# chrischoy/DeepGlobalRegistration

Hardware: NVIDIA H100
Metric: scan_pairs_per_sec (higher is better)
Workload: dtype f32

## Files before the change

deepglobalregistration_b200/csrc/spconv_ring.h:

```cpp
#pragma once

#if defined(__CUDACC__)
#define DGR_RING_HD __host__ __device__ __forceinline__
#else
#define DGR_RING_HD inline
#endif

namespace spconv_ring {

constexpr int kStages = 2;
constexpr int kIdxSlots = kStages + 1;
constexpr int kMaxRun = 8;

DGR_RING_HD int stage_of(unsigned g) { return (int)(g % kStages); }
DGR_RING_HD unsigned full_parity(unsigned g) { return (g / kStages) & 1u; }
DGR_RING_HD unsigned empty_parity(unsigned g) { return (g / kStages - 1u) & 1u; }
DGR_RING_HD int idx_slot(unsigned tile) { return (int)(tile % kIdxSlots); }

constexpr int kMinWaves = 2;
DGR_RING_HD int tile_run(int n_tiles, int resident) {
  const int r = n_tiles / (kMinWaves * (resident > 0 ? resident : 1));
  return r < 1 ? 1 : (r > kMaxRun ? kMaxRun : r);
}

}
```

deepglobalregistration_b200/csrc/spconv_tc.cu:

```cuda
#include <stdlib.h>

#include "common.cuh"
#include "spconv_ring.h"
#include "tc_common.cuh"

namespace {

using namespace tc;
using namespace spconv_ring;

#define DGR_TRY_RC(expr)             \
  do {                              \
    int32_t rc__ = (expr);          \
    if (rc__ != DGR_OK) return rc__; \
  } while (0)

constexpr int kConsumerWarps = 8;
constexpr int kProducerThreads = 128;
constexpr int kThreadsTC = kConsumerWarps * 32 + kProducerThreads;
constexpr int kTileM = 128;
constexpr int kChunk = 32;
constexpr int kATileBytes = kTileM * 128;
constexpr int kGatherRows = kTileM / (kProducerThreads / 8);
static_assert(kMaxRun <= 32, "one warp lists the tiles of a run");

struct TileDesc {
  int kappa, p0, rows;
};

struct TcShared {
  unsigned long long full[kStages];
  unsigned long long empty[kStages];
  int n_run;
  TileDesc tiles[kMaxRun];
  int out_rows[kIdxSlots][kTileM];
};

constexpr bool tc_line_epilogue(int nt) { return nt >= 128; }
constexpr int kScratchLd = 40;
constexpr int kScratchBytes = 16 * kScratchLd * 4;

constexpr size_t tc_smem_bytes(int nt) {
  return sizeof(TcShared) + 1024 + (size_t)kStages * (2 * kATileBytes + 2 * nt * 128) +
         (tc_line_epilogue(nt) ? (size_t)kConsumerWarps * kScratchBytes : 0);
}

constexpr int tc_min_ctas(int nt, bool f16) { return nt >= 128 || f16 ? 1 : 2; }
constexpr int kProducerRegs = 104, kConsumerRegs = 200;

template <int NT, bool kF16, int kPasses>
__global__ void __launch_bounds__(kThreadsTC, tc_min_ctas(NT, kF16))
spconv_tc_kernel(const float* __restrict__ in_feat, int cin, const unsigned char* __restrict__ wt, int cout,
                 const int32_t* __restrict__ in_idx, const int32_t* __restrict__ out_idx,
                 const int32_t* __restrict__ kofs, const int32_t* __restrict__ tile_k,
                 const int32_t* __restrict__ tile_start, int n_tiles, int run, const float* __restrict__ amax_in,
                 const float* __restrict__ w_inv_scale, float* __restrict__ out) {
  constexpr int kCh = kF16 ? 64 : kChunk;
  constexpr int kV = kF16 ? 2 : 1;
  constexpr int kBatches = kV, kBatchRows = kGatherRows / kBatches;
  constexpr int kBTileBytes = NT * 128;
  constexpr int kStageBytes = 2 * kATileBytes + 2 * kBTileBytes;
  extern __shared__ __align__(16) unsigned char smem_dyn[];
  TcShared& sh = *reinterpret_cast<TcShared*>(smem_dyn);
  unsigned char* stage0 = reinterpret_cast<unsigned char*>(
      (reinterpret_cast<uintptr_t>(smem_dyn) + sizeof(TcShared) + 1023) & ~(uintptr_t)1023);
  const int t = threadIdx.x, warp = __shfl_sync(0xffffffffu, t >> 5, 0), lane = t & 31;
  const int n_chunks = cin / kCh;
  const uint32_t b_tile_bytes = (uint32_t)cout * 128;
  const uint32_t slab_bytes = 2 * b_tile_bytes;
  const uint32_t full0 = smem_u32(&sh.full[0]), empty0 = smem_u32(&sh.empty[0]);

  if (t == 0) {
    for (int s = 0; s < kStages; ++s) {
      mbar_init(full0 + 8 * s, kProducerThreads + 1);
      mbar_init(empty0 + 8 * s, kConsumerWarps);
    }
    asm volatile("fence.mbarrier_init.release.cluster;" ::: "memory");
  }
  if (NT > cout) {
    const int pad_pieces = (NT - cout) * 8;
    for (int i = t; i < kStages * 2 * pad_pieces; i += kThreadsTC) {
      const int tile = i / pad_pieces, e = i % pad_pieces;
      *reinterpret_cast<uint4*>(stage0 + (tile >> 1) * kStageBytes + 2 * kATileBytes + (tile & 1) * kBTileBytes +
                                (cout + (e >> 3)) * 128 + (e & 7) * 16) = make_uint4(0u, 0u, 0u, 0u);
    }
  }
  if (warp == 0) {
    const int tile = blockIdx.x * run + lane;
    TileDesc d = {0, 0, 0};
    if (lane < run && tile < n_tiles) {
      d.kappa = tile_k[tile];
      d.p0 = tile_start[tile];
      d.rows = min(kTileM, kofs[d.kappa + 1] - d.p0);
    }
    const unsigned live = __ballot_sync(0xffffffffu, d.rows > 0);
    if (d.rows > 0) sh.tiles[__popc(live & ((1u << lane) - 1u))] = d;
    if (lane == 0) sh.n_run = __popc(live);
  }
  __syncthreads();
  const int n_run = sh.n_run;
  if (n_run == 0) return;

  if (warp >= kConsumerWarps) {
    if (NT >= 128) asm volatile("setmaxnreg.dec.sync.aligned.u32 %0;" ::"n"(kProducerRegs));
    const int pt = t - kConsumerWarps * 32, piece = pt & 7, rgrp = pt >> 3;
    const uint32_t a_off = (uint32_t)(rgrp * 128 + ((piece ^ (rgrp & 7)) << 4));
    const float sx = kF16 ? f16_scale_for(__ldg(amax_in)) : 1.f;
    auto load_idx = [&](int ti, int (&src)[kGatherRows], int& oj) {
      const TileDesc d = sh.tiles[ti < n_run ? ti : 0];
      const int rows = ti < n_run ? d.rows : 0;
#pragma unroll
      for (int i = 0; i < kGatherRows; ++i) {
        const int r = i * 16 + rgrp;
        src[i] = r < rows ? __ldg(in_idx + d.p0 + r) : -1;
      }
      oj = pt < rows ? __ldg(out_idx + d.p0 + pt) : -1;
    };
    int src[kGatherRows], src_next[kGatherRows], oj, oj_next;
    float4 v[kBatchRows][kV];
    auto load_a = [&](int c, int h) {
#pragma unroll
      for (int i = 0; i < kBatchRows; ++i)
#pragma unroll
        for (int u = 0; u < kV; ++u) {
          const int row = src[h * kBatchRows + i];
          v[i][u] = row >= 0 ? __ldg(reinterpret_cast<const float4*>(in_feat + (size_t)row * cin + c * kCh +
                                                                      piece * (4 * kV) + 4 * u))
                             : make_float4(0.f, 0.f, 0.f, 0.f);
        }
    };
    load_idx(0, src, oj);
    load_idx(1, src_next, oj_next);
    load_a(0, 0);
    unsigned g = 0;
    for (int ti = 0; ti < n_run; ++ti) {
      const unsigned char* slab = wt + (size_t)sh.tiles[ti].kappa * n_chunks * slab_bytes;
      for (int c = 0; c < n_chunks; ++c, ++g) {
        const int s = stage_of(g);
        unsigned char* a_hi = stage0 + (size_t)s * kStageBytes;
        unsigned char* a_lo = a_hi + kATileBytes;
        unsigned char* b_hi = a_lo + kATileBytes;
        if (g >= kStages) mbar_wait(empty0 + 8 * s, empty_parity(g));
        if (pt == 0) {
          const unsigned char* bsrc = slab + (size_t)c * slab_bytes;
          mbar_arrive_expect_tx(full0 + 8 * s, kPasses == 3 ? slab_bytes : b_tile_bytes);
          bulk_g2s(smem_u32(b_hi), bsrc, b_tile_bytes, full0 + 8 * s);
          if (kPasses == 3) bulk_g2s(smem_u32(b_hi + kBTileBytes), bsrc + b_tile_bytes, b_tile_bytes, full0 + 8 * s);
        }
        if (c == 0) sh.out_rows[idx_slot(ti)][pt] = oj;
#pragma unroll
        for (int h = 0; h < kBatches; ++h) {
#pragma unroll
          for (int i = 0; i < kBatchRows; ++i) {
            const uint32_t off = a_off + (h * kBatchRows + i) * 2048;
            if (kF16) split_store_f16(v[i][0], v[i][kV - 1], sx, a_hi, a_lo, off);
            else split_store(v[i][0], a_hi, a_lo, off);
          }
          if (h + 1 < kBatches) {
            load_a(c, h + 1);
          } else if (c + 1 < n_chunks) {
            load_a(c + 1, 0);
          } else if (ti + 1 < n_run) {
#pragma unroll
            for (int i = 0; i < kGatherRows; ++i) src[i] = src_next[i];
            oj = oj_next;
            load_a(0, 0);
            load_idx(ti + 2, src_next, oj_next);
          }
        }
        fence_proxy_async();
        mbar_arrive(full0 + 8 * s);
      }
    }
    return;
  }

  if (NT >= 128) asm volatile("setmaxnreg.inc.sync.aligned.u32 %0;" ::"n"(kConsumerRegs));
  const int wg = warp >> 2;
  const int r0 = wg * 64 + (warp & 3) * 16 + (lane >> 2);
  const float inv = kF16 ? __ldg(w_inv_scale) / f16_scale_for(__ldg(amax_in)) : 1.f;
  auto release = [&](unsigned gq) {
    __syncwarp();
    if (lane == 0) mbar_arrive(empty0 + 8 * stage_of(gq));
  };
  unsigned g = 0;
  for (int ti = 0; ti < n_run; ++ti) {
    float acc[NT / 2];
#pragma unroll
    for (int i = 0; i < NT / 2; ++i) acc[i] = 0.f;
    for (int c = 0; c < n_chunks; ++c, ++g) {
      const uint32_t a_hi = smem_u32(stage0 + (size_t)stage_of(g) * kStageBytes);
      const uint32_t b_hi = a_hi + 2 * kATileBytes;
      mbar_wait(full0 + 8 * stage_of(g), full_parity(g));
      wgmma_fence();
      const uint32_t a0 = a_hi + wg * (kATileBytes / 2);
      mma_chunk<NT, kF16, kPasses>(acc, a0, a0 + kATileBytes, b_hi, b_hi + kBTileBytes);
      wgmma_commit();
      wgmma_wait<1>();
      if (c > 0) release(g - 1);
    }
    wgmma_wait<0>();
    fence_acc(acc);
    release(g - 1);

    const int* rows_of = sh.out_rows[idx_slot(ti)];
    if constexpr (tc_line_epilogue(NT)) {
      float* scr = reinterpret_cast<float*>(stage0 + (size_t)kStages * kStageBytes + warp * kScratchBytes);
      const int lr = lane >> 2, lc = 2 * (lane & 3);
      const int sr = lane >> 3, sc = 4 * (lane & 7);
      int js[4];
#pragma unroll
      for (int k = 0; k < 4; ++k) js[k] = rows_of[r0 - lr + sr + 4 * k];
#pragma unroll
      for (int b = 0; b < NT / 32; ++b) {
        if (32 * b >= cout) break;
#pragma unroll
        for (int q = 0; q < 4; ++q) {
          const int i = 4 * b + q;
          *reinterpret_cast<float2*>(scr + lr * kScratchLd + 8 * q + lc) =
              make_float2(acc[4 * i] * inv, acc[4 * i + 1] * inv);
          *reinterpret_cast<float2*>(scr + (lr + 8) * kScratchLd + 8 * q + lc) =
              make_float2(acc[4 * i + 2] * inv, acc[4 * i + 3] * inv);
        }
        __syncwarp();
#pragma unroll
        for (int k = 0; k < 4; ++k) {
          const float4 v = *reinterpret_cast<const float4*>(scr + (sr + 4 * k) * kScratchLd + sc);
          if (js[k] >= 0 && 32 * b + sc < cout) red_add_v4(out + (size_t)js[k] * cout + 32 * b + sc, v.x, v.y, v.z, v.w);
        }
        __syncwarp();
      }
    } else {
      const int j0 = rows_of[r0], j1 = rows_of[r0 + 8];
      float* o0 = out + (size_t)(j0 < 0 ? 0 : j0) * cout;
      float* o1 = out + (size_t)(j1 < 0 ? 0 : j1) * cout;
#pragma unroll
      for (int i = 0; i < NT / 8; ++i) {
        const int col = 8 * i + 2 * (lane & 3);
        if (col < cout) {
          if (j0 >= 0) red_add_v2(o0 + col, acc[4 * i] * inv, acc[4 * i + 1] * inv);
          if (j1 >= 0) red_add_v2(o1 + col, acc[4 * i + 2] * inv, acc[4 * i + 3] * inv);
        }
      }
    }
  }
}

template <int NT, bool kF16, int kPasses>
int tc_resident_ctas(size_t smem) {
  int dev = 0, sms = 0, per_sm = 0;
  if (cudaGetDevice(&dev) != cudaSuccess ||
      cudaDeviceGetAttribute(&sms, cudaDevAttrMultiProcessorCount, dev) != cudaSuccess ||
      cudaOccupancyMaxActiveBlocksPerMultiprocessor(&per_sm, spconv_tc_kernel<NT, kF16, kPasses>, kThreadsTC, smem) !=
          cudaSuccess)
    return 0;
  return sms * per_sm;
}

template <int NT, bool kF16, int kPasses>
int32_t launch_spconv_tc(const float* in_feat, int cin, const void* wt, int cout, const int32_t* in_idx,
                         const int32_t* out_idx, const int32_t* kofs, const int32_t* tile_k, const int32_t* tile_start,
                         int n_tiles, const float* amax_in, const float* w_inv_scale, float* out, cudaStream_t st) {
  const size_t smem = tc_smem_bytes(NT);
  DGR_ENSURE_SMEM((spconv_tc_kernel<NT, kF16, kPasses>), smem);
  static const int resident = tc_resident_ctas<NT, kF16, kPasses>(smem);
  if (resident <= 0) {
    dgr_set_error("spconv_tc_kernel does not fit the device");
    return DGR_ERR_CUDA;
  }
  const int run = tile_run(n_tiles, resident);
  spconv_tc_kernel<NT, kF16, kPasses><<<(n_tiles + run - 1) / run, kThreadsTC, smem, st>>>(
      in_feat, cin, (const unsigned char*)wt, cout, in_idx, out_idx, kofs, tile_k, tile_start, n_tiles, run, amax_in,
      w_inv_scale, out);
  dgr_note_launches(1);
  DGR_LAUNCH_CHECK();
  return DGR_OK;
}

template <bool kF16, int kPasses>
int32_t launch_spconv_tc(const float* in_feat, int cin, const void* wt, int cout, const int32_t* in_idx,
                         const int32_t* out_idx, const int32_t* kofs, const int32_t* tile_k, const int32_t* tile_start,
                         int n_tiles, const float* amax_in, const float* w_inv_scale, float* out, cudaStream_t st) {
  auto launch = cout <= 32 ? launch_spconv_tc<32, kF16, kPasses> : cout <= 64 ? launch_spconv_tc<64, kF16, kPasses>
                : cout <= 128 ? launch_spconv_tc<128, kF16, kPasses> : launch_spconv_tc<256, kF16, kPasses>;
  return launch(in_feat, cin, wt, cout, in_idx, out_idx, kofs, tile_k, tile_start, n_tiles, amax_in, w_inv_scale, out, st);
}

__global__ void pack_weight_kernel(const float* __restrict__ w, int cin, int cout, float* __restrict__ packed) {
  const int n_chunks = cin / kChunk;
  const int64_t total = (int64_t)n_chunks * cout * 8;
  const int64_t e = (int64_t)blockIdx.x * blockDim.x + threadIdx.x;
  if (e >= total) return;
  const int kappa = blockIdx.y;
  const int n = (int)(e % cout);
  const int q = (int)((e / cout) % 8);
  const int ch = (int)(e / ((int64_t)cout * 8));
  const float* src = w + ((size_t)kappa * cin + ch * kChunk + q * 4) * cout + n;
  float4 v = make_float4(src[0], src[cout], src[2 * (size_t)cout], src[3 * (size_t)cout]);
  float4 h, l;
  h.x = tf32_round(v.x); h.y = tf32_round(v.y); h.z = tf32_round(v.z); h.w = tf32_round(v.w);
  l.x = v.x - h.x; l.y = v.y - h.y; l.z = v.z - h.z; l.w = v.w - h.w;
  float* slab = packed + ((size_t)kappa * n_chunks + ch) * 2 * cout * 32;
  const int off = n * 32 + ((q ^ (n & 7)) << 2);
  *reinterpret_cast<float4*>(slab + off) = h;
  *reinterpret_cast<float4*>(slab + (size_t)cout * 32 + off) = l;
}

__global__ void absmax_kernel(const float* __restrict__ x, int64_t n, unsigned* __restrict__ out) {
  float m = 0.f;
  const int64_t n4 = n >> 2;
  for (int64_t i = (int64_t)blockIdx.x * blockDim.x + threadIdx.x; i < n4; i += (int64_t)gridDim.x * blockDim.x) {
    const float4 v = __ldg(reinterpret_cast<const float4*>(x) + i);
    m = fmaxf(fmaxf(m, fmaxf(fabsf(v.x), fabsf(v.y))), fmaxf(fabsf(v.z), fabsf(v.w)));
  }
  if (blockIdx.x == 0 && threadIdx.x < (n & 3)) m = fmaxf(m, fabsf(x[(n4 << 2) + threadIdx.x]));
#pragma unroll
  for (int d = 16; d > 0; d >>= 1) m = fmaxf(m, __shfl_xor_sync(0xffffffffu, m, d));
  if ((threadIdx.x & 31) == 0 && m > 0.f) atomicMax(out, __float_as_uint(m));
}

__global__ void pack_weight_f16_kernel(const float* __restrict__ w, int cin, int cout, const float* __restrict__ amax,
                                       unsigned char* __restrict__ packed, float* __restrict__ scale) {
  const int n_chunks = cin / 64;
  const int64_t total = (int64_t)n_chunks * cout * 8;
  const int64_t e = (int64_t)blockIdx.x * blockDim.x + threadIdx.x;
  const float sw = f16_scale_for(*amax);
  if (e == 0 && blockIdx.y == 0) scale[0] = 1.f / sw;
  if (e >= total) return;
  const int kappa = blockIdx.y;
  const int n = (int)(e % cout);
  const int q = (int)((e / cout) % 8);
  const int ch = (int)(e / ((int64_t)cout * 8));
  const float* src = w + ((size_t)kappa * cin + ch * 64 + q * 8) * cout + n;
  uint32_t h[4], l[4];
#pragma unroll
  for (int i = 0; i < 4; ++i) {
    const float x0 = src[(size_t)(2 * i) * cout] * sw, x1 = src[(size_t)(2 * i + 1) * cout] * sw;
    const __half2 hh = __floats2half2_rn(x0, x1);
    const float2 hf = __half22float2(hh);
    const __half2 ll = __floats2half2_rn(x0 - hf.x, x1 - hf.y);
    h[i] = *reinterpret_cast<const uint32_t*>(&hh);
    l[i] = *reinterpret_cast<const uint32_t*>(&ll);
  }
  unsigned char* slab = packed + ((size_t)kappa * n_chunks + ch) * 2 * cout * 128;
  const int off = n * 128 + ((q ^ (n & 7)) << 4);
  *reinterpret_cast<uint4*>(slab + off) = make_uint4(h[0], h[1], h[2], h[3]);
  *reinterpret_cast<uint4*>(slab + (size_t)cout * 128 + off) = make_uint4(l[0], l[1], l[2], l[3]);
}

}

extern "C" {

int32_t dgr_pack_weight_tf32(const float* w, int32_t K, int32_t cin, int32_t cout, float* packed, void* stream) {
  DGR_ARG_CHECK(K >= 1 && cin >= 32 && cin % 32 == 0 && cout >= 8 && cout % 8 == 0, "bad weight shape");
  DGR_ARG_CHECK(K <= 65535, "K too large");
  const int64_t per_k = (int64_t)(cin / kChunk) * cout * 8;
  dim3 grid(dgr_blocks(per_k, 256), K);
  pack_weight_kernel<<<grid, 256, 0, (cudaStream_t)stream>>>(w, cin, cout, packed);
  dgr_note_launches(1);
  DGR_LAUNCH_CHECK();
  return DGR_OK;
}


int32_t dgr_spconv_tc_supported(int32_t cin, int32_t cout) {
  return (cin >= 32 && cin % 32 == 0 && cout >= 16 && cout <= 256 && cout % 16 == 0) ? 1 : 0;
}

int32_t dgr_spconv_tc_fwd(const float* in_feat, int32_t cin, const float* weight_t, int32_t cout,
                          const int32_t* in_idx, const int32_t* out_idx, const int32_t* kofs,
                          const int32_t* tile_k, const int32_t* tile_start, int32_t n_tiles,
                          int32_t tile_rows, int32_t passes, float* out, void* stream) {
  DGR_ARG_CHECK(tile_rows == kTileM, "tile_rows must be 128");
  DGR_ARG_CHECK(dgr_spconv_tc_supported(cin, cout), "shape not supported by the tensor-core path");
  DGR_ARG_CHECK(passes == 1 || passes == 3, "passes must be 1 or 3");
  DGR_ARG_CHECK(((uintptr_t)out & 15) == 0, "out must be 16-byte aligned");
  if (n_tiles == 0) return DGR_OK;
  auto launch = passes == 3 ? launch_spconv_tc<false, 3> : launch_spconv_tc<false, 1>;
  return launch(in_feat, cin, weight_t, cout, in_idx, out_idx, kofs, tile_k, tile_start, n_tiles, nullptr, nullptr, out,
                (cudaStream_t)stream);
}

int32_t dgr_absmax_f32(const float* x, int64_t n, float* amax, void* stream) {
  cudaStream_t st = (cudaStream_t)stream;
  DGR_CUDA_CHECK(cudaMemsetAsync(amax, 0, sizeof(float), st));
  if (n <= 0) return DGR_OK;
  int dev = 0, sms = 0;
  DGR_CUDA_CHECK(cudaGetDevice(&dev));
  DGR_CUDA_CHECK(cudaDeviceGetAttribute(&sms, cudaDevAttrMultiProcessorCount, dev));
  unsigned blocks = dgr_blocks(n / 4 + 1, 256);
  if (blocks > 4u * sms) blocks = 4u * sms;
  absmax_kernel<<<blocks, 256, 0, st>>>(x, n, reinterpret_cast<unsigned*>(amax));
  dgr_note_launches(1);
  DGR_LAUNCH_CHECK();
  return DGR_OK;
}

int32_t dgr_spconv_tc_f16_supported(int32_t cin, int32_t cout) {
  return (cin >= 64 && cin % 64 == 0 && cout >= 32 && cout <= 256 && cout % 32 == 0) ? 1 : 0;
}

int32_t dgr_pack_weight_f16(const float* w, int32_t K, int32_t cin, int32_t cout, void* packed, float* scale_ws,
                            void* stream) {
  DGR_ARG_CHECK(K >= 1 && K <= 65535 && dgr_spconv_tc_f16_supported(cin, cout), "bad weight shape");
  DGR_TRY_RC(dgr_absmax_f32(w, (int64_t)K * cin * cout, scale_ws + 1, stream));
  const int64_t per_k = (int64_t)(cin / 64) * cout * 8;
  dim3 grid(dgr_blocks(per_k, 256), K);
  pack_weight_f16_kernel<<<grid, 256, 0, (cudaStream_t)stream>>>(w, cin, cout, scale_ws + 1, (unsigned char*)packed,
                                                               scale_ws);
  dgr_note_launches(1);
  DGR_LAUNCH_CHECK();
  return DGR_OK;
}

int32_t dgr_spconv_tc_f16_fwd(const float* in_feat, int32_t cin, const void* weight_h, int32_t cout,
                              const int32_t* in_idx, const int32_t* out_idx, const int32_t* kofs,
                              const int32_t* tile_k, const int32_t* tile_start, int32_t n_tiles, int32_t tile_rows,
                              const float* amax_in, const float* w_scale, float* out, void* stream) {
  DGR_ARG_CHECK(tile_rows == kTileM, "tile_rows must be 128");
  DGR_ARG_CHECK(dgr_spconv_tc_f16_supported(cin, cout), "shape not supported by the 3xFP16 path");
  DGR_ARG_CHECK(amax_in != nullptr && w_scale != nullptr, "scales missing");
  DGR_ARG_CHECK(((uintptr_t)out & 15) == 0, "out must be 16-byte aligned");
  if (n_tiles == 0) return DGR_OK;
  return launch_spconv_tc<true, 3>(in_feat, cin, weight_h, cout, in_idx, out_idx, kofs, tile_k, tile_start, n_tiles,
                                   amax_in, w_scale, out, (cudaStream_t)stream);
}

}
```

Before: 81.09.

## Add ping-pong warpgroup sparse conv kernel for wide f16 layers

Adds a new sparse-convolution kernel in which two consumer warpgroups alternate over 64-row half-tiles in ping-pong order. Four producer warps each own one stage of a four-stage A ring, and the whole weight slab for a kernel offset is kept resident in shared memory. Output columns are split into 128-wide halves across CTAs, and results are scattered through a per-warp scratch buffer as vector atomic adds. The aim is to overlap one warpgroup's epilogue with the other's MMAs and to reuse weights across tiles; the cost is a more complex barrier protocol, a single CTA per SM, and recomputing the A gather for each column half.

Result: faster. 82.48 (median of 6 runs) (+1.7%).

```diff
diff --git a/deepglobalregistration_b200/csrc/spconv_ring.h b/deepglobalregistration_b200/csrc/spconv_ring.h
--- a/deepglobalregistration_b200/csrc/spconv_ring.h
+++ b/deepglobalregistration_b200/csrc/spconv_ring.h
@@ -12,10 +12,21 @@
 constexpr int kIdxSlots = kStages + 1;
 constexpr int kMaxRun = 8;
 
-DGR_RING_HD int stage_of(unsigned g) { return (int)(g % kStages); }
-DGR_RING_HD unsigned full_parity(unsigned g) { return (g / kStages) & 1u; }
-DGR_RING_HD unsigned empty_parity(unsigned g) { return (g / kStages - 1u) & 1u; }
+template <int S>
+struct Ring {
+  static DGR_RING_HD int stage(unsigned g) { return (int)(g % S); }
+  static DGR_RING_HD unsigned full_parity(unsigned g) { return (g / S) & 1u; }
+  static DGR_RING_HD unsigned empty_parity(unsigned g) { return (g / S - 1u) & 1u; }
+  static DGR_RING_HD unsigned retired_parity(unsigned g) { return (g / S) & 1u; }
+};
+
+DGR_RING_HD int stage_of(unsigned g) { return Ring<kStages>::stage(g); }
+DGR_RING_HD unsigned full_parity(unsigned g) { return Ring<kStages>::full_parity(g); }
+DGR_RING_HD unsigned empty_parity(unsigned g) { return Ring<kStages>::empty_parity(g); }
 DGR_RING_HD int idx_slot(unsigned tile) { return (int)(tile % kIdxSlots); }
+
+constexpr int kPpStages = 4;
+using PpRing = Ring<kPpStages>;
 
 constexpr int kMinWaves = 2;
 DGR_RING_HD int tile_run(int n_tiles, int resident) {
diff --git a/deepglobalregistration_b200/csrc/spconv_tc.cu b/deepglobalregistration_b200/csrc/spconv_tc.cu
--- a/deepglobalregistration_b200/csrc/spconv_tc.cu
+++ b/deepglobalregistration_b200/csrc/spconv_tc.cu
@@ -246,15 +246,243 @@
   }
 }
 
-template <int NT, bool kF16, int kPasses>
-int tc_resident_ctas(size_t smem) {
+constexpr int kPpCols = 128;
+constexpr int kPpRows = 64;
+constexpr int kPpMaxChunks = 4;
+constexpr int kPpMaxHalves = 2 * kMaxRun;
+constexpr int kPpAStageBytes = 2 * kPpRows * 128;
+constexpr int kPpBChunkBytes = 2 * kPpCols * 128;
+static_assert(kPpMaxHalves <= 32, "one warp lists the half-tiles of a run");
+
+struct HalfDesc {
+  int kappa, p0, rows;
+  int use;
+};
+
+struct PpShared {
+  unsigned long long full[kPpStages];
+  unsigned long long empty[kPpStages];
+  unsigned long long b_full[kPpMaxChunks];
+  unsigned long long order[2];
+  int n_half;
+  HalfDesc half[kPpMaxHalves];
+  int in_rows[kPpMaxHalves * kPpRows];
+  int out_rows[kPpMaxHalves * kPpRows];
+};
+
+constexpr size_t pp_smem_bytes() {
+  return sizeof(PpShared) + 1024 + (size_t)kPpMaxChunks * kPpBChunkBytes + (size_t)kPpStages * kPpAStageBytes +
+         (size_t)kConsumerWarps * kScratchBytes;
+}
+static_assert(pp_smem_bytes() <= 227 * 1024, "an sm_90 block holds at most 227 KB of shared memory");
+
+constexpr int kPpProducerRegs = 232, kPpConsumerRegs = 136;
+static_assert(kPpStages * 32 == kProducerThreads, "one producer warp per ring stage");
+__global__ void __launch_bounds__(kThreadsTC, 1)
+spconv_pp_kernel(const float* __restrict__ in_feat, int cin, const unsigned char* __restrict__ wt, int cout,
+                 const int32_t* __restrict__ in_idx, const int32_t* __restrict__ out_idx,
+                 const int32_t* __restrict__ kofs, const int32_t* __restrict__ tile_k,
+                 const int32_t* __restrict__ tile_start, int n_tiles, int run, const float* __restrict__ amax_in,
+                 const float* __restrict__ w_inv_scale, float* __restrict__ out) {
+  extern __shared__ __align__(16) unsigned char smem_dyn[];
+  PpShared& sh = *reinterpret_cast<PpShared*>(smem_dyn);
+  unsigned char* b_base = reinterpret_cast<unsigned char*>(
+      (reinterpret_cast<uintptr_t>(smem_dyn) + sizeof(PpShared) + 1023) & ~(uintptr_t)1023);
+  unsigned char* a_base = b_base + kPpMaxChunks * kPpBChunkBytes;
+  unsigned char* scr_base = a_base + kPpStages * kPpAStageBytes;
+  const int t = threadIdx.x, warp = __shfl_sync(0xffffffffu, t >> 5, 0), lane = t & 31;
+  const int halves = (cout + kPpCols - 1) / kPpCols;
+  const int col0 = (int)(blockIdx.x % halves) * kPpCols, ncols = min(kPpCols, cout - col0);
+  const int first_tile = (int)(blockIdx.x / halves) * run;
+  const int n_chunks = cin / 64;
+  const uint32_t b_tile_bytes = (uint32_t)ncols * 128;
+  const uint32_t full0 = smem_u32(&sh.full[0]), empty0 = smem_u32(&sh.empty[0]);
+  const uint32_t b_full0 = smem_u32(&sh.b_full[0]), order0 = smem_u32(&sh.order[0]);
+
+  if (t == 0) {
+    for (int s = 0; s < kPpStages; ++s) {
+      mbar_init(full0 + 8 * s, 32);
+      mbar_init(empty0 + 8 * s, kConsumerWarps / 2);
+    }
+    for (int c = 0; c < kPpMaxChunks; ++c) mbar_init(b_full0 + 8 * c, 1);
+    for (int w = 0; w < 2; ++w) mbar_init(order0 + 8 * w, kConsumerWarps / 2);
+    asm volatile("fence.mbarrier_init.release.cluster;" ::: "memory");
+  }
+  if (ncols < kPpCols) {
+    const int pad_pieces = (kPpCols - ncols) * 8;
+    for (int i = t; i < 2 * kPpMaxChunks * pad_pieces; i += kThreadsTC) {
+      const int tile = i / pad_pieces, e = i % pad_pieces;
+      *reinterpret_cast<uint4*>(b_base + tile * (kPpBChunkBytes / 2) + (ncols + (e >> 3)) * 128 + (e & 7) * 16) =
+          make_uint4(0u, 0u, 0u, 0u);
+    }
+  }
+  if (warp == 0) {
+    const int ti = lane >> 1, hf = lane & 1, tile = first_tile + ti;
+    HalfDesc d = {0, 0, 0, 0};
+    if (ti < run && tile < n_tiles) {
+      d.kappa = tile_k[tile];
+      d.p0 = tile_start[tile] + hf * kPpRows;
+      d.rows = min(kPpRows, kofs[d.kappa + 1] - d.p0);
+    }
+    const unsigned live = __ballot_sync(0xffffffffu, d.rows > 0);
+    const int n = __popc(live);
+    if (d.rows > 0) sh.half[__popc(live & ((1u << lane) - 1u))] = d;
+    __syncwarp();
+    const unsigned change =
+        __ballot_sync(0xffffffffu, lane > 0 && lane < n && sh.half[lane].kappa != sh.half[lane - 1].kappa);
+    if (lane < n) sh.half[lane].use = __popc(change & ((2u << lane) - 1u));
+    if (lane == 0) sh.n_half = n;
+  }
+  __syncthreads();
+  const int n_half = sh.n_half;
+  if (n_half == 0) return;
+
+  auto load_slab = [&](int kappa) {
+    for (int c = 0; c < n_chunks; ++c) {
+      const unsigned char* src = wt + ((size_t)kappa * n_chunks + c) * 2 * cout * 128 + (size_t)col0 * 128;
+      unsigned char* dst = b_base + c * kPpBChunkBytes;
+      const uint32_t bar = b_full0 + 8 * c;
+      mbar_arrive_expect_tx(bar, 2 * b_tile_bytes);
+      bulk_g2s(smem_u32(dst), src, b_tile_bytes, bar);
+      bulk_g2s(smem_u32(dst + kPpBChunkBytes / 2), src + (size_t)cout * 128, b_tile_bytes, bar);
+    }
+  };
+  const int producer0 = kConsumerWarps * 32;
+  if (t == producer0) load_slab(sh.half[0].kappa);
+  for (int e = t; e < n_half * kPpRows; e += kThreadsTC) {
+    const HalfDesc d = sh.half[e / kPpRows];
+    const int r = e % kPpRows;
+    sh.in_rows[e] = r < d.rows ? __ldg(in_idx + d.p0 + r) : -1;
+    sh.out_rows[e] = r < d.rows ? __ldg(out_idx + d.p0 + r) : -1;
+  }
+  fence_proxy_async();
+  __syncthreads();
+
+  if (warp >= kConsumerWarps) {
+    asm volatile("setmaxnreg.inc.sync.aligned.u32 %0;" ::"n"(kPpProducerRegs));
+    const int pw = warp - kConsumerWarps, piece = lane & 7, rsub = lane >> 3;
+    const float sx = f16_scale_for(__ldg(amax_in));
+    const unsigned n_g = (unsigned)(n_half * n_chunks);
+    unsigned char* a_hi = a_base + pw * kPpAStageBytes;
+    float4 v[kPpRows / 4][2];
+    for (unsigned g = (unsigned)pw; g < n_g; g += kPpStages) {
+      const int i = (int)(g / n_chunks), c = (int)(g - (unsigned)i * n_chunks);
+#pragma unroll
+      for (int k = 0; k < kPpRows / 4; ++k) {
+        const int row = sh.in_rows[i * kPpRows + rsub + 4 * k];
+        const float4* src = reinterpret_cast<const float4*>(in_feat + (size_t)row * cin + c * 64 + piece * 8);
+#pragma unroll
+        for (int u = 0; u < 2; ++u) v[k][u] = row >= 0 ? __ldg(src + u) : make_float4(0.f, 0.f, 0.f, 0.f);
+      }
+      if (c == 0 && i > 0 && sh.half[i].use != sh.half[i - 1].use) {
+        for (unsigned q = g > (unsigned)kPpStages ? g - kPpStages : 0u; q < g; ++q)
+          mbar_wait(empty0 + 8 * PpRing::stage(q), PpRing::retired_parity(q));
+        if (lane == 0) load_slab(sh.half[i].kappa);
+      }
+      if (g >= (unsigned)kPpStages) mbar_wait(empty0 + 8 * pw, PpRing::empty_parity(g));
+#pragma unroll
+      for (int k = 0; k < kPpRows / 4; ++k) {
+        const int r = rsub + 4 * k;
+        split_store_f16(v[k][0], v[k][1], sx, a_hi, a_hi + kPpAStageBytes / 2,
+                        (uint32_t)(r * 128 + ((piece ^ (r & 7)) << 4)));
+      }
+      fence_proxy_async();
+      mbar_arrive(full0 + 8 * pw);
+    }
+    return;
+  }
+
+  asm volatile("setmaxnreg.dec.sync.aligned.u32 %0;" ::"n"(kPpConsumerRegs));
+  const int wg = warp >> 2;
+  const float inv = __ldg(w_inv_scale) / f16_scale_for(__ldg(amax_in));
+  float* scr = reinterpret_cast<float*>(scr_base + warp * kScratchBytes);
+  const int lr = lane >> 2, lc = 2 * (lane & 3);
+  const int sr = lane >> 3, sc = 4 * (lane & 7);
+  auto release = [&](unsigned gq) {
+    __syncwarp();
+    if (lane == 0) mbar_arrive(empty0 + 8 * PpRing::stage(gq));
+  };
+  unsigned k = 0;
+  for (int i = wg; i < n_half; i += 2, ++k) {
+    if (k + wg > 0) mbar_wait(order0 + 8 * wg, (k + wg - 1) & 1u);
+    const unsigned use_parity = (unsigned)sh.half[i].use & 1u;
+    float acc[kPpCols / 2];
+#pragma unroll
+    for (int e = 0; e < kPpCols / 2; ++e) acc[e] = 0.f;
+    unsigned g = (unsigned)(i * n_chunks);
+    for (int c = 0; c < n_chunks; ++c, ++g) {
+      const uint32_t a_hi = smem_u32(a_base + PpRing::stage(g) * kPpAStageBytes);
+      const uint32_t b_hi = smem_u32(b_base + c * kPpBChunkBytes);
+      mbar_wait(b_full0 + 8 * c, use_parity);
+      mbar_wait(full0 + 8 * PpRing::stage(g), PpRing::full_parity(g));
+      wgmma_fence();
+      mma_chunk<kPpCols, true, 3>(acc, a_hi, a_hi + kPpAStageBytes / 2, b_hi, b_hi + kPpBChunkBytes / 2);
+      wgmma_commit();
+      if (c + 1 == n_chunks) {
+        __syncwarp();
+        if (lane == 0) mbar_arrive(order0 + 8 * (wg ^ 1));
+      }
+      wgmma_wait<1>();
+      if (c > 0) release(g - 1);
+    }
+    wgmma_wait<0>();
+    fence_acc(acc);
+    release(g - 1);
+
+    const int* rows_of = sh.out_rows + i * kPpRows + (warp & 3) * 16;
+    int js[4];
+#pragma unroll
+    for (int q = 0; q < 4; ++q) js[q] = rows_of[sr + 4 * q];
+#pragma unroll
+    for (int b = 0; b < kPpCols / 32; ++b) {
+      if (32 * b >= ncols) break;
+#pragma unroll
+      for (int q = 0; q < 4; ++q) {
+        const int e = 4 * b + q;
+        *reinterpret_cast<float2*>(scr + lr * kScratchLd + 8 * q + lc) =
+            make_float2(acc[4 * e] * inv, acc[4 * e + 1] * inv);
+        *reinterpret_cast<float2*>(scr + (lr + 8) * kScratchLd + 8 * q + lc) =
+            make_float2(acc[4 * e + 2] * inv, acc[4 * e + 3] * inv);
+      }
+      __syncwarp();
+#pragma unroll
+      for (int q = 0; q < 4; ++q) {
+        const float4 v = *reinterpret_cast<const float4*>(scr + (sr + 4 * q) * kScratchLd + sc);
+        if (js[q] >= 0) red_add_v4(out + (size_t)js[q] * cout + col0 + 32 * b + sc, v.x, v.y, v.z, v.w);
+      }
+      __syncwarp();
+    }
+  }
+}
+
+template <class Kernel>
+int tc_resident_ctas(Kernel kernel, size_t smem) {
   int dev = 0, sms = 0, per_sm = 0;
   if (cudaGetDevice(&dev) != cudaSuccess ||
       cudaDeviceGetAttribute(&sms, cudaDevAttrMultiProcessorCount, dev) != cudaSuccess ||
-      cudaOccupancyMaxActiveBlocksPerMultiprocessor(&per_sm, spconv_tc_kernel<NT, kF16, kPasses>, kThreadsTC, smem) !=
-          cudaSuccess)
+      cudaOccupancyMaxActiveBlocksPerMultiprocessor(&per_sm, kernel, kThreadsTC, smem) != cudaSuccess)
     return 0;
   return sms * per_sm;
+}
+
+int32_t launch_spconv_pp(const float* in_feat, int cin, const void* wt, int cout, const int32_t* in_idx,
+                         const int32_t* out_idx, const int32_t* kofs, const int32_t* tile_k, const int32_t* tile_start,
+                         int n_tiles, const float* amax_in, const float* w_inv_scale, float* out, cudaStream_t st) {
+  const size_t smem = pp_smem_bytes();
+  DGR_ENSURE_SMEM(spconv_pp_kernel, smem);
+  static const int resident = tc_resident_ctas(spconv_pp_kernel, smem);
+  if (resident <= 0) {
+    dgr_set_error("spconv_pp_kernel does not fit the device");
+    return DGR_ERR_CUDA;
+  }
+  const int halves = (cout + kPpCols - 1) / kPpCols;
+  const int run = tile_run(n_tiles * halves, resident);
+  spconv_pp_kernel<<<(n_tiles + run - 1) / run * halves, kThreadsTC, smem, st>>>(
+      in_feat, cin, (const unsigned char*)wt, cout, in_idx, out_idx, kofs, tile_k, tile_start, n_tiles, run, amax_in,
+      w_inv_scale, out);
+  dgr_note_launches(1);
+  DGR_LAUNCH_CHECK();
+  return DGR_OK;
 }
 
 template <int NT, bool kF16, int kPasses>
@@ -263,7 +491,7 @@
                          int n_tiles, const float* amax_in, const float* w_inv_scale, float* out, cudaStream_t st) {
   const size_t smem = tc_smem_bytes(NT);
   DGR_ENSURE_SMEM((spconv_tc_kernel<NT, kF16, kPasses>), smem);
-  static const int resident = tc_resident_ctas<NT, kF16, kPasses>(smem);
+  static const int resident = tc_resident_ctas(spconv_tc_kernel<NT, kF16, kPasses>, smem);
   if (resident <= 0) {
     dgr_set_error("spconv_tc_kernel does not fit the device");
     return DGR_ERR_CUDA;
@@ -281,6 +509,9 @@
 int32_t launch_spconv_tc(const float* in_feat, int cin, const void* wt, int cout, const int32_t* in_idx,
                          const int32_t* out_idx, const int32_t* kofs, const int32_t* tile_k, const int32_t* tile_start,
                          int n_tiles, const float* amax_in, const float* w_inv_scale, float* out, cudaStream_t st) {
+  if (kF16 && cout > 64 && cin <= 64 * kPpMaxChunks)
+    return launch_spconv_pp(in_feat, cin, wt, cout, in_idx, out_idx, kofs, tile_k, tile_start, n_tiles, amax_in,
+                            w_inv_scale, out, st);
   auto launch = cout <= 32 ? launch_spconv_tc<32, kF16, kPasses> : cout <= 64 ? launch_spconv_tc<64, kF16, kPasses>
                 : cout <= 128 ? launch_spconv_tc<128, kF16, kPasses> : launch_spconv_tc<256, kF16, kPasses>;
   return launch(in_feat, cin, wt, cout, in_idx, out_idx, kofs, tile_k, tile_start, n_tiles, amax_in, w_inv_scale, out, st);
```
